# tzt101/MichiGAN

Hardware: NVIDIA H100
Metric: 512x512 images/sec (generator forward) (higher is better)
Workload: dtype fp16/bf16 tensor-core operands (bf16 hi+lo split where needed), fp32 accumulate and storage

## Files before the change

michigan_b200/csrc/mg_aux.cu:

```cuda
#include <cuda_runtime.h>
#include <cstdint>
#include <cmath>
#include <cstdlib>
#include <cuda_fp16.h>
#include <cuda_bf16.h>
#include "mg_internal.h"

namespace mg {

__device__ __forceinline__ float rtf32(float x) {
    uint32_t r;
    asm("cvt.rna.tf32.f32 %0, %1;\n" : "=r"(r) : "f"(x));
    return __uint_as_float(r);
}
__device__ __forceinline__ float act_fn(float v, int act) {
    if (act == MG_ACT_RELU) return fmaxf(v, 0.f);
    if (act == MG_ACT_LRELU) return v > 0.f ? v : 0.2f * v;
    if (act == MG_ACT_TANH) return tanhf(v);
    return v;
}
__device__ __forceinline__ void split16(float v, int fmt, uint16_t& hi, uint16_t& lo) {
    if (fmt == 1) {
        const __half h = __float2half_rn(fminf(fmaxf(v, -65504.f), 65504.f));
        hi = __half_as_ushort(h);
        lo = __half_as_ushort(__float2half_rn(v - __half2float(h)));
    } else {
        const __nv_bfloat16 h = __float2bfloat16_rn(v);
        hi = __bfloat16_as_ushort(h);
        lo = __bfloat16_as_ushort(__float2bfloat16_rn(v - __bfloat162float(h)));
    }
}
static inline int cdiv(long long a, long long b) { return (int)((a + b - 1) / b); }

__global__ void pack_weight_kernel(const float* __restrict__ w, float* __restrict__ out, int O, int I, int KH, int KW,
                                   const float* __restrict__ inv_sigma, int round_) {
    const long long total = (long long)O * KH * KW * I;
    const float s = inv_sigma ? *inv_sigma : 1.f;
    for (long long idx = blockIdx.x * (long long)blockDim.x + threadIdx.x; idx < total;
         idx += (long long)gridDim.x * blockDim.x) {
        const int i = idx % I;
        long long t = idx / I;
        const int kw = t % KW; t /= KW;
        const int kh = t % KH;
        const int o = t / KH;
        float v = w[(((long long)o * I + i) * KH + kh) * KW + kw] * s;
        out[idx] = round_ ? rtf32(v) : v;
    }
}

__global__ void pack_weight_gb_kernel(const float* __restrict__ wg, const float* __restrict__ wb,
                                      float* __restrict__ out, int C, int I, int KH, int KW, int BN) {
    const long long total = 2LL * C * KH * KW * I;
    const int half = BN / 2;
    for (long long idx = blockIdx.x * (long long)blockDim.x + threadIdx.x; idx < total;
         idx += (long long)gridDim.x * blockDim.x) {
        const int i = idx % I;
        long long t = idx / I;
        const int kw = t % KW; t /= KW;
        const int kh = t % KH;
        const int R = t / KH;
        const int tile = R / BN, rr = R % BN;
        const float* src = rr < half ? wg : wb;
        const int c = tile * half + (rr < half ? rr : rr - half);
        out[idx] = rtf32(src[(((long long)c * I + i) * KH + kh) * KW + kw]);
    }
}

__global__ void pack_weight16_kernel(const float* __restrict__ w, uint16_t* __restrict__ out, int O, int I, int KH, int KW,
                                     const float* __restrict__ inv_sigma, int fmt, int split) {
    const long long total = (long long)O * KH * KW * I;
    const float s = inv_sigma ? *inv_sigma : 1.f;
    const int parts = split ? 2 : 1;
    for (long long idx = blockIdx.x * (long long)blockDim.x + threadIdx.x; idx < total;
         idx += (long long)gridDim.x * blockDim.x) {
        const int i = idx % I;
        long long t = idx / I;
        const int kw = t % KW; t /= KW;
        const int kh = t % KH;
        const int o = t / KH;
        const float v = w[(((long long)o * I + i) * KH + kh) * KW + kw] * s;
        uint16_t hi, lo;
        split16(v, fmt, hi, lo);
        const size_t base = ((size_t)o * KH * KW + (size_t)(kh * KW + kw)) * parts * I;
        out[base + i] = hi;
        if (split) out[base + I + i] = lo;
    }
}
__global__ void pack_weight_gb16_kernel(const float* __restrict__ wg, const float* __restrict__ wb, uint16_t* __restrict__ out,
                                        int C, int I, int KH, int KW, int BN, int fmt, int split) {
// ... 109 lines not shown
                            }
                        }
#pragma unroll
                        for (int p_ = 0; p_ < 8; ++p_) {
                            const float* ip = row + (size_t)(((g * 8 + p_) * s + kw)) * CINP;
                            float iv[CINP];
                            const float4 t0 = *reinterpret_cast<const float4*>(ip);
                            iv[0] = t0.x; iv[1] = t0.y; iv[2] = t0.z; iv[3] = t0.w;
                            if constexpr (CINP == 8) {
                                const float4 t1 = *reinterpret_cast<const float4*>(ip + 4);
                                iv[4] = t1.x; iv[5] = t1.y; iv[6] = t1.z; iv[7] = t1.w;
                            }
#pragma unroll
                            for (int ci = 0; ci < CINP; ++ci)
#pragma unroll
                                for (int c = 0; c < CPL; ++c) acc[p_][c] = fmaf(iv[ci], wv[ci][c], acc[p_][c]);
                        }
                    }
                }
            }
            if (lane_active && oh < a.OH) {
                float bv[CPL];
#pragma unroll
                for (int c = 0; c < CPL; ++c) bv[c] = a.bias ? __ldg(a.bias + c_base + c) : 0.f;
#pragma unroll
                for (int p_ = 0; p_ < 8; ++p_) {
                    const int ow = ow0 + g * 8 + p_;
                    if (ow >= a.OW) continue;
                    const size_t pix = ((size_t)n * a.OH + oh) * a.OW + ow;
                    const float ps = a.pscale ? __ldg(a.pscale + pix) : 1.f;
                    const float pm = a.pmul ? __ldg(a.pmul + pix) : 1.f;
                    float y[CPL];
#pragma unroll
                    for (int c = 0; c < CPL; ++c) {
                        float v = act_fn(acc[p_][c] * ps + bv[c], a.act) * pm;
                        y[c] = a.round_out ? rtf32(v) : v;
                    }
                    if (a.out) {
                        float* op = a.out + pix * Cout + c_base;
                        if constexpr (CPL == 4) *reinterpret_cast<float4*>(op) = make_float4(y[0], y[1], y[2], y[3]);
                        else *reinterpret_cast<float2*>(op) = make_float2(y[0], y[1]);
                    }
                    if (a.out_hi) {
                        uint16_t hi[CPL], lo[CPL];
#pragma unroll
                        for (int c = 0; c < CPL; ++c) split16(y[c], a.out16_fmt, hi[c], lo[c]);
                        uint16_t* oh = reinterpret_cast<uint16_t*>(a.out_hi) + pix * Cout + c_base;
                        uint16_t* ol = a.out_lo ? reinterpret_cast<uint16_t*>(a.out_lo) + pix * Cout + c_base : nullptr;
                        if constexpr (CPL == 4) {
                            *reinterpret_cast<uint2*>(oh) = make_uint2(hi[0] | ((uint32_t)hi[1] << 16), hi[2] | ((uint32_t)hi[3] << 16));
                            if (ol) *reinterpret_cast<uint2*>(ol) = make_uint2(lo[0] | ((uint32_t)lo[1] << 16), lo[2] | ((uint32_t)lo[3] << 16));
                        } else {
                            *reinterpret_cast<uint32_t*>(oh) = hi[0] | ((uint32_t)hi[1] << 16);
                            if (ol) *reinterpret_cast<uint32_t*>(ol) = lo[0] | ((uint32_t)lo[1] << 16);
                        }
                    }
                }
            }
        }
    }
}


template <int CINP, int CPT>
__global__ void __launch_bounds__(256, 1)
thin_gemm_kernel(const mg_thin_args a, int tiles_w, int tiles_h, int num_tiles) {
    extern __shared__ __align__(16) float sm[];
    const int KH = a.KH, KW = a.KW, s = a.stride;
    constexpr int Cout = 16 * CPT;
    const int PH = 7 * s + KH, PW = 15 * s + KW;
    float* w_s = sm;
    float* in_s = sm + KH * KW * CINP * Cout;
    const int nw = KH * KW * CINP * Cout;
    for (int i = threadIdx.x * 4; i < nw; i += blockDim.x * 4)
        *reinterpret_cast<float4*>(w_s + i) = __ldg(reinterpret_cast<const float4*>(a.w + i));
    const int tx = threadIdx.x & 15, ty = threadIdx.x >> 4;
    const int prow = ty >> 1, pcol0 = (ty & 1) * 8;
    const int c_base = tx * CPT;
    const int R = a.seg_resize > 0 ? a.seg_resize : 1;
    const int IH = a.H, IW = a.W;
    float bv[CPT];
#pragma unroll
    for (int c = 0; c < CPT; ++c) bv[c] = a.bias ? __ldg(a.bias + c_base + c) : 0.f;

    for (int tile = blockIdx.x; tile < num_tiles; tile += gridDim.x) {
        const int tw = tile % tiles_w;
        const int th = (tile / tiles_w) % tiles_h;
        const int n = tile / (tiles_w * tiles_h);
        const int oh0 = th * 8, ow0 = tw * 16;
        const int ih0 = oh0 * s - a.pad, iw0 = ow0 * s - a.pad;
        __syncthreads();
        for (int i = threadIdx.x; i < PH * PW; i += blockDim.x) {
            const int py = i / PW, px = i - py * PW;
            int ih = ih0 + py, iw = iw0 + px;
            if (a.pad_mode == 1) {
                if (ih < 0) ih = -ih;
                if (ih >= IH) ih = 2 * IH - 2 - ih;
                if (iw < 0) iw = -iw;
                if (iw >= IW) iw = 2 * IW - 2 - iw;
            }
            const bool ok = ih >= 0 && ih < IH && iw >= 0 && iw < IW;
            float4 v0 = make_float4(0.f, 0.f, 0.f, 0.f), v1 = v0;
            if (ok) {
                const float* src = a.in + (((size_t)n * IH * R + (size_t)ih * R) * ((size_t)IW * R) + (size_t)iw * R) * CINP;
                v0 = __ldg(reinterpret_cast<const float4*>(src));
                if (CINP == 8) v1 = __ldg(reinterpret_cast<const float4*>(src + 4));
            }
            *reinterpret_cast<float4*>(in_s + (size_t)i * CINP) = v0;
            if (CINP == 8) *reinterpret_cast<float4*>(in_s + (size_t)i * CINP + 4) = v1;
        }
        __syncthreads();

        float acc[8][CPT];
#pragma unroll
        for (int p_ = 0; p_ < 8; ++p_)
#pragma unroll
            for (int c = 0; c < CPT; ++c) acc[p_][c] = 0.f;
        for (int kh = 0; kh < KH; ++kh) {
            const float* row = in_s + (size_t)((prow * s + kh) * PW) * CINP;
            for (int kw = 0; kw < KW; ++kw) {
                const float* wt = w_s + (size_t)((kh * KW + kw) * CINP) * Cout + c_base;
#pragma unroll
                for (int c4 = 0; c4 < CINP; c4 += 4) {
                    float wv[4][CPT];
#pragma unroll
                    for (int ci = 0; ci < 4; ++ci)
#pragma unroll
                        for (int c = 0; c < CPT; c += 4) {
                            const float4 t = *reinterpret_cast<const float4*>(wt + (size_t)(c4 + ci) * Cout + c);
                            wv[ci][c] = t.x; wv[ci][c + 1] = t.y; wv[ci][c + 2] = t.z; wv[ci][c + 3] = t.w;
                        }
#pragma unroll
                    for (int p_ = 0; p_ < 8; ++p_) {
                        const float4 iv = *reinterpret_cast<const float4*>(row + (size_t)((pcol0 + p_) * s + kw) * CINP + c4);
#pragma unroll
                        for (int c = 0; c < CPT; ++c) {
                            acc[p_][c] = fmaf(iv.x, wv[0][c], acc[p_][c]);
                            acc[p_][c] = fmaf(iv.y, wv[1][c], acc[p_][c]);
                            acc[p_][c] = fmaf(iv.z, wv[2][c], acc[p_][c]);
                            acc[p_][c] = fmaf(iv.w, wv[3][c], acc[p_][c]);
                        }
                    }
                }
            }
        }
        const int oh = oh0 + prow;
        if (oh < a.OH) {
#pragma unroll
            for (int p_ = 0; p_ < 8; ++p_) {
                const int ow = ow0 + pcol0 + p_;
                if (ow >= a.OW) continue;
                const size_t pix = ((size_t)n * a.OH + oh) * a.OW + ow;
                const float ps = a.pscale ? __ldg(a.pscale + pix) : 1.f;
                const float pm = a.pmul ? __ldg(a.pmul + pix) : 1.f;
                float y[CPT];
#pragma unroll
                for (int c = 0; c < CPT; ++c) {
                    const float v = act_fn(acc[p_][c] * ps + bv[c], a.act) * pm;
                    y[c] = a.round_out ? rtf32(v) : v;
                }
                if (a.out) {
                    float* op = a.out + pix * Cout + c_base;
#pragma unroll
                    for (int c = 0; c < CPT; c += 4) *reinterpret_cast<float4*>(op + c) = make_float4(y[c], y[c + 1], y[c + 2], y[c + 3]);
                }
                if (a.out_hi) {
                    uint16_t hi[CPT], lo[CPT];
#pragma unroll
                    for (int c = 0; c < CPT; ++c) split16(y[c], a.out16_fmt, hi[c], lo[c]);
                    uint16_t* ohp = reinterpret_cast<uint16_t*>(a.out_hi) + pix * Cout + c_base;
                    uint16_t* olp = a.out_lo ? reinterpret_cast<uint16_t*>(a.out_lo) + pix * Cout + c_base : nullptr;
#pragma unroll
                    for (int c = 0; c < CPT; c += 4) {
                        *reinterpret_cast<uint2*>(ohp + c) = make_uint2(hi[c] | ((uint32_t)hi[c + 1] << 16), hi[c + 2] | ((uint32_t)hi[c + 3] << 16));
                        if (olp) *reinterpret_cast<uint2*>(olp + c) = make_uint2(lo[c] | ((uint32_t)lo[c + 1] << 16), lo[c + 2] | ((uint32_t)lo[c + 3] << 16));
                    }
                }
            }
        }
    }
}

__global__ void __launch_bounds__(256)
conv_img_kernel(const float* __restrict__ x, const float* __restrict__ w, const float* __restrict__ bias,
                float* __restrict__ out, int N, int H, int W, int Cin, int Cout, int act_in, int act_out) {
    extern __shared__ __align__(16) float sm[];
    const int PW = 34, PH = 10, NP = PW * PH;
    const int C4 = Cin / 4;
    float* in_s = sm;
    float* w_s = sm + (size_t)C4 * NP * 4;
    for (int i = threadIdx.x; i < 9 * Cin * 4; i += blockDim.x) {
        const int co = i & 3;
        const int ci = (i >> 2) % Cin;
        const int tap = (i >> 2) / Cin;
        w_s[i] = co < Cout ? w[((size_t)co * Cin + ci) * 9 + tap] : 0.f;
    }
    const int tiles_w = (W + 31) / 32, tiles_h = (H + 7) / 8;
    const int tile = blockIdx.x;
    const int tw = tile % tiles_w, th = (tile / tiles_w) % tiles_h, n = tile / (tiles_w * tiles_h);
    const int h0 = th * 8 - 1, w0 = tw * 32 - 1;
    for (int i0 = threadIdx.x; i0 < NP * C4; i0 += 4 * blockDim.x) {
        float4 v[4];
#pragma unroll
        for (int u = 0; u < 4; ++u) {
            const int i = i0 + u * blockDim.x;
            const int c4 = i % C4, pp = i / C4;
            const int py = pp / PW, px = pp - py * PW;
            const int ih = h0 + py, iw = w0 + px;
            v[u] = make_float4(0.f, 0.f, 0.f, 0.f);
            if (i < NP * C4 && ih >= 0 && ih < H && iw >= 0 && iw < W)
                v[u] = __ldg(reinterpret_cast<const float4*>(x + (((size_t)n * H + ih) * W + iw) * Cin) + c4);
        }
#pragma unroll
        for (int u = 0; u < 4; ++u) {
            const int i = i0 + u * blockDim.x;
            if (i >= NP * C4) break;
            const int c4 = i % C4, pp = i / C4;
            const float4 r = make_float4(act_fn(v[u].x, act_in), act_fn(v[u].y, act_in), act_fn(v[u].z, act_in), act_fn(v[u].w, act_in));
            *reinterpret_cast<float4*>(in_s + ((size_t)c4 * NP + pp) * 4) = r;
        }
    }
    __syncthreads();
    const int ly = threadIdx.x >> 5, lx = threadIdx.x & 31;
    float a0 = 0.f, a1 = 0.f, a2 = 0.f;
    for (int kh = 0; kh < 3; ++kh)
        for (int kw = 0; kw < 3; ++kw) {
            const int pp = (ly + kh) * PW + lx + kw;
            const float* wt = w_s + (size_t)((kh * 3 + kw) * Cin) * 4;
// ... 863 lines not shown
```

michigan_b200/csrc/mg_wgrad.cu:

```cuda
#include <cuda.h>
#include <cuda_runtime.h>
#include <cstdio>
#include <cstring>
#include <cstdlib>
#include "mg_ptx.cuh"
#include "mg_internal.h"

namespace mg {

constexpr int kWgThreads = 288;
constexpr int kWgStagesMax = 6;
constexpr int kWgMaxCols = 256;

struct WgradParams {
    int N, OH, OW, Cout, Cin, KH, KW, stride, pad;
    int TW, TH, TN, tiles_w, tiles_h, tiles_n, pix_tiles;
    int BN, m_tiles, n_tiles, splits, stages;
    int pix_tile, box_bytes;
    int f16;
    int kelem, mboxes, kmma;
    float* dw;
    double* dw64;
};

__device__ __forceinline__ uint32_t sw128(uint32_t k, uint32_t b) {
    const uint32_t o = k * 128 + b;
    return o ^ ((k & 7) << 4);
}

__device__ __forceinline__ void mma_tf32_16x8x8(float (&c)[4], const uint32_t (&a)[4], uint32_t b0, uint32_t b1) {
    asm volatile("mma.sync.aligned.m16n8k8.row.col.f32.tf32.tf32.f32 {%0, %1, %2, %3}, {%4, %5, %6, %7}, {%8, %9}, {%0, %1, %2, %3};\n"
                 : "+f"(c[0]), "+f"(c[1]), "+f"(c[2]), "+f"(c[3])
                 : "r"(a[0]), "r"(a[1]), "r"(a[2]), "r"(a[3]), "r"(b0), "r"(b1));
}
__device__ __forceinline__ void mma_bf16_16x8x16(float (&c)[4], const uint32_t (&a)[4], uint32_t b0, uint32_t b1) {
    asm volatile("mma.sync.aligned.m16n8k16.row.col.f32.bf16.bf16.f32 {%0, %1, %2, %3}, {%4, %5, %6, %7}, {%8, %9}, {%0, %1, %2, %3};\n"
                 : "+f"(c[0]), "+f"(c[1]), "+f"(c[2]), "+f"(c[3])
                 : "r"(a[0]), "r"(a[1]), "r"(a[2]), "r"(a[3]), "r"(b0), "r"(b1));
}

template <int KWT, int BNT>
__global__ void __launch_bounds__(kWgThreads, 1)
wgrad_tf32_kernel(const __grid_constant__ CUtensorMap tmDY, const __grid_constant__ CUtensorMap tmX, const WgradParams p) {
    extern __shared__ __align__(1024) uint8_t smem_raw[];
    uint8_t* smem = reinterpret_cast<uint8_t*>((reinterpret_cast<uintptr_t>(smem_raw) + 1023) & ~uintptr_t(1023));
    const int kBoxBytes = p.box_bytes;
    const int a_bytes = p.mboxes * kBoxBytes;
    const int b1_bytes = (p.BN / p.kelem) * kBoxBytes;
    const int stage_bytes = a_bytes + p.KW * b1_bytes;
    uint64_t* bars = reinterpret_cast<uint64_t*>(smem + (size_t)p.stages * stage_bytes);
    uint64_t* full_bar = bars;
    uint64_t* empty_bar = bars + kWgStagesMax;

    const int warp = threadIdx.x >> 5, lane = threadIdx.x & 31;
    const int n_units = p.KH * p.m_tiles * p.n_tiles;
    int u = blockIdx.x % n_units;
    const int split = blockIdx.x / n_units;
    const int nt = u % p.n_tiles; u /= p.n_tiles;
    const int mt = u % p.m_tiles;
    const int kh = u / p.m_tiles;
    const int t_begin = (int)((long long)p.pix_tiles * split / p.splits);
    const int t_end = (int)((long long)p.pix_tiles * (split + 1) / p.splits);

    if (warp == 8 && lane == 0) {
        tma_prefetch_desc(&tmDY);
        tma_prefetch_desc(&tmX);
        for (int s = 0; s < p.stages; ++s) { mbar_init(&full_bar[s], 1); mbar_init(&empty_bar[s], 8); }
        fence_barrier_init();
    }
    __syncthreads();

    if (warp == 8) {
        int st = 0; uint32_t ph = 0;
        const int nb_x = p.BN / p.kelem;
        const uint32_t tx = (uint32_t)stage_bytes;
        const int n_boxes = p.mboxes + p.KW * nb_x;
        for (int t = t_begin; t < t_end; ++t) {
            const int tw = t % p.tiles_w;
            const int th = (t / p.tiles_w) % p.tiles_h;
            const int tn = t / (p.tiles_w * p.tiles_h);
            const int ow0 = tw * p.TW, oh0 = th * p.TH, n0 = tn * p.TN;
            if (lane == 0) {
                mbar_wait_report(&empty_bar[st], ph ^ 1);
                mbar_arrive_expect_tx(&full_bar[st], tx);
            }
            __syncwarp();
            uint8_t* sa = smem + (size_t)st * stage_bytes;
            for (int b = lane; b < n_boxes; b += 32) {
                if (b < p.mboxes) {
                    tma_load_4d(sa + b * kBoxBytes, &tmDY, &full_bar[st], mt * 128 + b * p.kelem, ow0, oh0, n0);
                } else {
                    const int kw = (b - p.mboxes) / nb_x, j = (b - p.mboxes) - kw * nb_x;
                    tma_load_4d(sa + a_bytes + kw * b1_bytes + j * kBoxBytes, &tmX, &full_bar[st], nt * p.BN + j * p.kelem,
                                ow0 * p.stride - p.pad + kw, oh0 * p.stride - p.pad + kh, n0);
                }
            }
            __syncwarp();
            if (++st == p.stages) { st = 0; ph ^= 1; }
        }
    } else if constexpr (KWT > 0) {
        const int wg = warp >> 2;
        float acc[KWT][BNT / 2];
#pragma unroll
        for (int kw = 0; kw < KWT; ++kw)
#pragma unroll
            for (int i = 0; i < BNT / 2; ++i) acc[kw][i] = 0.f;
        int st = 0; uint32_t ph = 0;
        for (int t = t_begin; t < t_end; ++t) {
            mbar_wait(&full_bar[st], ph);
            const uint32_t sa = smem_u32(smem + (size_t)st * stage_bytes);
            const uint32_t a_base = sa + (uint32_t)(wg * kBoxBytes), b_base = sa + (uint32_t)a_bytes;
            wgmma_fence();
#pragma unroll 1
            for (int kk = 0; kk < p.pix_tile; kk += 16) {
                const uint64_t da = wg_desc_mn_sw128(a_base + (uint32_t)(kk * 128), (uint32_t)kBoxBytes);
#pragma unroll
                for (int kw = 0; kw < KWT; ++kw) {
                    const uint64_t db = wg_desc_mn_sw128(b_base + (uint32_t)(kw * b1_bytes + kk * 128), (uint32_t)kBoxBytes);
                    if constexpr (BNT == 128) wgmma_bf16_tt_n128(acc[kw], da, db, 1u);
                    else wgmma_bf16_tt_n64(acc[kw], da, db, 1u);
                }
            }
            wgmma_commit();
            wgmma_wait_all();
            __syncwarp();
            if (lane == 0) mbar_arrive(&empty_bar[st]);
            if (++st == p.stages) { st = 0; ph ^= 1; }
        }
        if (t_end > t_begin) {
            const int r0 = mt * 128 + wg * 64 + (warp & 3) * 16 + (lane >> 2), c0 = (lane & 3) * 2;
#pragma unroll
            for (int h = 0; h < 2; ++h) {
                const int co = r0 + 8 * h;
                if (co >= p.Cout) continue;
#pragma unroll
                for (int kw = 0; kw < KWT; ++kw)
#pragma unroll
                    for (int j = 0; j < BNT / 8; ++j) {
                        const size_t off = (size_t)co * (p.KH * KWT * p.Cin) + (size_t)(kh * KWT + kw) * p.Cin + nt * BNT + j * 8 + c0;
                        const float v0 = acc[kw][4 * j + 2 * h], v1 = acc[kw][4 * j + 2 * h + 1];
                        if (p.splits > 1) {
                            atomicAdd(p.dw64 + off, (double)v0);
                            atomicAdd(p.dw64 + off + 1, (double)v1);
                        } else {
                            *reinterpret_cast<float2*>(p.dw + off) = make_float2(v0, v1);
                        }
                    }
            }
        }
    } else {
        const int g = lane >> 2, t4 = lane & 3;
        const int m0 = warp * 16;
        const int ncols = p.KW * p.BN, n8 = ncols >> 3;
        const int esz = p.f16 ? 2 : 4;
        uint32_t a_off[2];
#pragma unroll
        for (int h = 0; h < 2; ++h) {
            const int m = m0 + g + 8 * h;
            a_off[h] = (uint32_t)((m / p.kelem) * kBoxBytes) | ((uint32_t)((m % p.kelem) * esz) << 20);
        }
        float acc[kWgMaxCols / 8][4];
#pragma unroll
        for (int j = 0; j < kWgMaxCols / 8; ++j) acc[j][0] = acc[j][1] = acc[j][2] = acc[j][3] = 0.f;
        int st = 0; uint32_t ph = 0;
        for (int t = t_begin; t < t_end; ++t) {
            mbar_wait(&full_bar[st], ph);
            const uint8_t* sa = smem + (size_t)st * stage_bytes;
            auto ldA = [&](int h, int k) -> const uint8_t* { return sa + (a_off[h] & 0xFFFFF) + sw128(k, a_off[h] >> 20); };
            for (int kk = 0; kk < p.pix_tile; kk += p.kmma) {
                uint32_t a[4];
                if (p.f16) {
#pragma unroll
                    for (int i = 0; i < 4; ++i) {
                        const int h = i & 1, k = kk + 2 * t4 + 8 * (i >> 1);
                        a[i] = (uint32_t)*reinterpret_cast<const uint16_t*>(ldA(h, k)) |
                               ((uint32_t)*reinterpret_cast<const uint16_t*>(ldA(h, k + 1)) << 16);
                    }
                } else {
#pragma unroll
                    for (int i = 0; i < 4; ++i) a[i] = *reinterpret_cast<const uint32_t*>(ldA(i & 1, kk + t4 + 4 * (i >> 1)));
                }
#pragma unroll
                for (int j = 0; j < kWgMaxCols / 8; ++j) {
                    if (j < n8) {
                        const int n = j * 8 + g, kw = n / p.BN, ci = n - kw * p.BN;
                        const uint8_t* bb = sa + a_bytes + kw * b1_bytes + (ci / p.kelem) * kBoxBytes;
                        const uint32_t cb = (uint32_t)((ci % p.kelem) * esz);
                        if (p.f16) {
                            const int k = kk + 2 * t4;
                            const uint32_t b0 = (uint32_t)*reinterpret_cast<const uint16_t*>(bb + sw128(k, cb)) |
                                                ((uint32_t)*reinterpret_cast<const uint16_t*>(bb + sw128(k + 1, cb)) << 16);
                            const uint32_t b1 = (uint32_t)*reinterpret_cast<const uint16_t*>(bb + sw128(k + 8, cb)) |
                                                ((uint32_t)*reinterpret_cast<const uint16_t*>(bb + sw128(k + 9, cb)) << 16);
                            mma_bf16_16x8x16(acc[j], a, b0, b1);
                        } else {
                            const uint32_t b0 = *reinterpret_cast<const uint32_t*>(bb + sw128(kk + t4, cb));
                            const uint32_t b1 = *reinterpret_cast<const uint32_t*>(bb + sw128(kk + t4 + 4, cb));
                            mma_tf32_16x8x8(acc[j], a, b0, b1);
                        }
                    }
                }
            }
            __syncwarp();
            if (lane == 0) mbar_arrive(&empty_bar[st]);
            if (++st == p.stages) { st = 0; ph ^= 1; }
        }
        if (t_end > t_begin) {
#pragma unroll
            for (int h = 0; h < 2; ++h) {
                const int co = mt * 128 + m0 + g + 8 * h;
                if (co >= p.Cout) continue;
#pragma unroll
                for (int j = 0; j < kWgMaxCols / 8; ++j) {
                    if (j < n8) {
                        const int n = j * 8 + 2 * t4, kw = n / p.BN, ci = n - kw * p.BN;
                        const size_t off = (size_t)co * (p.KH * p.KW * p.Cin) + (size_t)(kh * p.KW + kw) * p.Cin + nt * p.BN + ci;
                        if (p.splits > 1) {
                            atomicAdd(p.dw64 + off, (double)acc[j][2 * h]);
                            atomicAdd(p.dw64 + off + 1, (double)acc[j][2 * h + 1]);
                        } else {
                            *reinterpret_cast<float2*>(p.dw + off) = make_float2(acc[j][2 * h], acc[j][2 * h + 1]);
                        }
                    }
                }
            }
        }
    }
}

static int np2(int v) { int r = 1; while (r < v) r <<= 1; return r; }

}

using namespace mg;

static int wgrad_launch(const void* dy, const void* x, float* dw, int N, int H, int W, int Cin, int OH, int OW, int Cout,
                        int KH, int KW, int stride, int pad, int fmt, cudaStream_t stream) {
    if (!dy || !x || !dw) return set_error(-1, "mg_conv_wgrad: null pointer");
    if (fmt != 0 && fmt != 2) return set_error(-5, "mg_conv_wgrad: operand format must be 0 (tf32) or 2 (bf16)");
    const int kelem = fmt ? 64 : 32;
    if (Cin % kelem != 0 || Cout % kelem != 0) return set_error(-2, "mg_conv_wgrad: channels must be multiples of %d", kelem);
    WgradParams p;
    memset(&p, 0, sizeof(p));
    p.N = N; p.OH = OH; p.OW = OW; p.Cout = Cout; p.Cin = Cin; p.KH = KH; p.KW = KW; p.stride = stride; p.pad = pad;
    p.f16 = fmt; p.kelem = kelem; p.mboxes = 128 / kelem; p.kmma = fmt ? 16 : 8;
    int BN = Cin >= 128 ? 128 : Cin;
    if (Cin % BN != 0) BN = kelem;
    while (KW * BN > kWgMaxCols) BN /= 2;
    if (BN < kelem || Cin % BN != 0) return set_error(-3, "mg_conv_wgrad: KW %d x Cin %d does not fit the accumulator", KW, Cin);
    p.BN = BN;
    int pix_tile = 64;
    if ((200 * 1024) / ((p.mboxes + KW * (BN / kelem)) * 64 * 128) < 3) pix_tile = 32;
    p.pix_tile = pix_tile; p.box_bytes = pix_tile * 128;
    p.TW = np2(OW) < 8 ? np2(OW) : 8;
    int th = pix_tile / p.TW;
    p.TH = np2(OH) < th ? np2(OH) : th;
    p.TN = pix_tile / (p.TW * p.TH);
    p.tiles_w = (OW + p.TW - 1) / p.TW; p.tiles_h = (OH + p.TH - 1) / p.TH; p.tiles_n = (N + p.TN - 1) / p.TN;
    p.pix_tiles = p.tiles_w * p.tiles_h * p.tiles_n;
    p.m_tiles = (Cout + 127) / 128;
    p.n_tiles = Cin / BN;
    const int units = KH * p.m_tiles * p.n_tiles;
    int splits = (2 * num_sms()) / units;
    if (splits < 1) splits = 1;
    if (splits > p.pix_tiles) splits = p.pix_tiles;
    p.splits = splits;
    const int stage_bytes = p.mboxes * p.box_bytes + KW * (BN / kelem) * p.box_bytes;
    int stages = (200 * 1024) / stage_bytes;
    if (stages < 1) return set_error(-4, "mg_conv_wgrad: stage of %d bytes does not fit shared memory", stage_bytes);
    if (stages > kWgStagesMax) stages = kWgStagesMax;
    p.stages = stages;
    p.dw = dw;

    CUtensorMap tmDY, tmX;
    const int esz = fmt ? 2 : 4;
    const CUtensorMapDataType dt = fmt ? CU_TENSOR_MAP_DATA_TYPE_BFLOAT16 : CU_TENSOR_MAP_DATA_TYPE_FLOAT32;
    const CUtensorMapSwizzle sw = CU_TENSOR_MAP_SWIZZLE_128B;
    {
        cuuint64_t dims[4] = {(cuuint64_t)Cout, (cuuint64_t)OW, (cuuint64_t)OH, (cuuint64_t)N};
        cuuint64_t strides[3] = {(cuuint64_t)Cout * esz, (cuuint64_t)OW * Cout * esz, (cuuint64_t)OH * OW * Cout * esz};
        cuuint32_t box[4] = {(cuuint32_t)kelem, (cuuint32_t)p.TW, (cuuint32_t)p.TH, (cuuint32_t)p.TN};
        cuuint32_t es[4] = {1, 1, 1, 1};
        int rc = encode_tensor_map(&tmDY, (void*)dy, dt, 4, dims, strides, box, es, sw);
        if (rc) return rc;
    }
    {
        cuuint64_t dims[4] = {(cuuint64_t)Cin, (cuuint64_t)W, (cuuint64_t)H, (cuuint64_t)N};
        cuuint64_t strides[3] = {(cuuint64_t)Cin * esz, (cuuint64_t)W * Cin * esz, (cuuint64_t)H * W * Cin * esz};
        cuuint32_t box[4] = {(cuuint32_t)kelem, (cuuint32_t)(p.TW * stride), (cuuint32_t)(p.TH * stride), (cuuint32_t)p.TN};
        cuuint32_t es[4] = {1, (cuuint32_t)stride, (cuuint32_t)stride, 1};
        int rc = encode_tensor_map(&tmX, (void*)x, dt, 4, dims, strides, box, es, sw);
        if (rc) return rc;
    }
    void (*kern)(CUtensorMap, CUtensorMap, WgradParams) = wgrad_tf32_kernel<0, 0>;
    if (fmt == 2) {
        if (KW == 1 && BN == 64) kern = wgrad_tf32_kernel<1, 64>;
        else if (KW == 1 && BN == 128) kern = wgrad_tf32_kernel<1, 128>;
        else if (KW == 2 && BN == 64) kern = wgrad_tf32_kernel<2, 64>;
        else if (KW == 2 && BN == 128) kern = wgrad_tf32_kernel<2, 128>;
        else if (KW == 3 && BN == 64) kern = wgrad_tf32_kernel<3, 64>;
        else if (KW == 4 && BN == 64) kern = wgrad_tf32_kernel<4, 64>;
    }
    cudaError_t e = cudaFuncSetAttribute((const void*)kern, cudaFuncAttributeMaxDynamicSharedMemorySize, 227 * 1024);
    if (e != cudaSuccess) return set_error((int)e, "wgrad attr: %s", cudaGetErrorString(e));
    const size_t smem_bytes = (size_t)stages * stage_bytes + 1024 + 256;
    const size_t n_dw = (size_t)Cout * KH * KW * Cin;
    if (splits > 1) {
        const int rc = acc64_alloc(&p.dw64, n_dw, stream);
        if (rc) return rc;
    }
    kern<<<units * splits, kWgThreads, smem_bytes, stream>>>(tmDY, tmX, p);
    int rc = check_launch("mg_conv_wgrad");
    if (splits > 1) {
        if (!rc) rc = acc64_fold(p.dw64, dw, n_dw, 0, stream);
        const int rc2 = acc64_free(p.dw64, stream);
        if (!rc) rc = rc2;
    }
    return rc;
}

extern "C" int mg_conv_wgrad(const float* dy, const float* x, float* dw, int N, int H, int W, int Cin, int OH, int OW, int Cout,
                             int KH, int KW, int stride, int pad, void* stream_) {
    return wgrad_launch(dy, x, dw, N, H, W, Cin, OH, OW, Cout, KH, KW, stride, pad, 0, reinterpret_cast<cudaStream_t>(stream_));
}

extern "C" int mg_conv_wgrad16(const void* dy16, const void* x16, float* dw, int N, int H, int W, int Cin, int OH, int OW, int Cout,
                               int KH, int KW, int stride, int pad, void* stream_) {
    return wgrad_launch(dy16, x16, dw, N, H, W, Cin, OH, OW, Cout, KH, KW, stride, pad, 2, reinterpret_cast<cudaStream_t>(stream_));
}
```

Before: 201.7.

## Skip zero last input channel in thin conv and move TF32 wgrad to wgmma

The thin direct-convolution kernel now checks whether the last padded input channel's weights are all zero and, if so, runs a compile-time variant that skips those FMAs. Separately, the TF32 weight-gradient kernel replaces its mma.sync fallback with a wgmma path: TMA lands tiles in a ring, and consumer warps transpose them into double-buffered K-major stages before issuing wgmma. The wgrad change only matters for backward passes, so it probably does not affect the generator-forward metric. It adds shared-memory transposes, and it fails with an error for any KW/BN combination that has no compiled variant.

```diff
diff --git a/michigan_b200/csrc/mg_aux.cu b/michigan_b200/csrc/mg_aux.cu
--- a/michigan_b200/csrc/mg_aux.cu
+++ b/michigan_b200/csrc/mg_aux.cu
@@ -5,6 +5,7 @@
 #include <cuda_fp16.h>
 #include <cuda_bf16.h>
 #include "mg_internal.h"
+#include <type_traits>
 
 namespace mg {
 
@@ -280,6 +281,12 @@
     float bv[CPT];
 #pragma unroll
     for (int c = 0; c < CPT; ++c) bv[c] = a.bias ? __ldg(a.bias + c_base + c) : 0.f;
+    bool last_nz = false;
+    for (int i = threadIdx.x; i < KH * KW * Cout; i += blockDim.x) {
+        const int tap = i / Cout, c = i - tap * Cout;
+        last_nz |= __ldg(a.w + (size_t)(tap * CINP + CINP - 1) * Cout + c) != 0.f;
+    }
+    const bool skip_last = !__syncthreads_or(last_nz);
 
     for (int tile = blockIdx.x; tile < num_tiles; tile += gridDim.x) {
         const int tw = tile % tiles_w;
@@ -314,34 +321,39 @@
         for (int p_ = 0; p_ < 8; ++p_)
 #pragma unroll
             for (int c = 0; c < CPT; ++c) acc[p_][c] = 0.f;
-        for (int kh = 0; kh < KH; ++kh) {
-            const float* row = in_s + (size_t)((prow * s + kh) * PW) * CINP;
-            for (int kw = 0; kw < KW; ++kw) {
-                const float* wt = w_s + (size_t)((kh * KW + kw) * CINP) * Cout + c_base;
-#pragma unroll
-                for (int c4 = 0; c4 < CINP; c4 += 4) {
-                    float wv[4][CPT];
-#pragma unroll
-                    for (int ci = 0; ci < 4; ++ci)
-#pragma unroll
-                        for (int c = 0; c < CPT; c += 4) {
-                            const float4 t = *reinterpret_cast<const float4*>(wt + (size_t)(c4 + ci) * Cout + c);
-                            wv[ci][c] = t.x; wv[ci][c + 1] = t.y; wv[ci][c + 2] = t.z; wv[ci][c + 3] = t.w;
-                        }
-#pragma unroll
-                    for (int p_ = 0; p_ < 8; ++p_) {
-                        const float4 iv = *reinterpret_cast<const float4*>(row + (size_t)((pcol0 + p_) * s + kw) * CINP + c4);
-#pragma unroll
-                        for (int c = 0; c < CPT; ++c) {
-                            acc[p_][c] = fmaf(iv.x, wv[0][c], acc[p_][c]);
-                            acc[p_][c] = fmaf(iv.y, wv[1][c], acc[p_][c]);
-                            acc[p_][c] = fmaf(iv.z, wv[2][c], acc[p_][c]);
-                            acc[p_][c] = fmaf(iv.w, wv[3][c], acc[p_][c]);
+        auto mac = [&](auto nci) {
+            constexpr int NCI = decltype(nci)::value;
+            for (int kh = 0; kh < KH; ++kh) {
+                const float* row = in_s + (size_t)((prow * s + kh) * PW) * CINP;
+                for (int kw = 0; kw < KW; ++kw) {
+                    const float* wt = w_s + (size_t)((kh * KW + kw) * CINP) * Cout + c_base;
+#pragma unroll
+                    for (int c4 = 0; c4 < CINP; c4 += 4) {
+                        float wv[4][CPT];
+#pragma unroll
+                        for (int ci = 0; ci < 4; ++ci)
+#pragma unroll
+                            for (int c = 0; c < CPT; c += 4) {
+                                if (c4 + ci >= NCI) continue;
+                                const float4 t = *reinterpret_cast<const float4*>(wt + (size_t)(c4 + ci) * Cout + c);
+                                wv[ci][c] = t.x; wv[ci][c + 1] = t.y; wv[ci][c + 2] = t.z; wv[ci][c + 3] = t.w;
+                            }
+#pragma unroll
+                        for (int p_ = 0; p_ < 8; ++p_) {
+                            const float4 iv = *reinterpret_cast<const float4*>(row + (size_t)((pcol0 + p_) * s + kw) * CINP + c4);
+                            const float ivs[4] = {iv.x, iv.y, iv.z, iv.w};
+#pragma unroll
+                            for (int c = 0; c < CPT; ++c)
+#pragma unroll
+                                for (int ci = 0; ci < 4; ++ci)
+                                    if (c4 + ci < NCI) acc[p_][c] = fmaf(ivs[ci], wv[ci][c], acc[p_][c]);
                         }
                     }
                 }
             }
-        }
+        };
+        if (skip_last) mac(std::integral_constant<int, CINP - 1>{});
+        else mac(std::integral_constant<int, CINP>{});
         const int oh = oh0 + prow;
         if (oh < a.OH) {
 #pragma unroll
diff --git a/michigan_b200/csrc/mg_wgrad.cu b/michigan_b200/csrc/mg_wgrad.cu
--- a/michigan_b200/csrc/mg_wgrad.cu
+++ b/michigan_b200/csrc/mg_wgrad.cu
@@ -11,54 +11,69 @@
 constexpr int kWgThreads = 288;
 constexpr int kWgStagesMax = 6;
 constexpr int kWgMaxCols = 256;
+constexpr int kWgSmemBudget = 200 * 1024;
+constexpr int kWgTf32Box = 32 * 128;
 
 struct WgradParams {
-    int N, OH, OW, Cout, Cin, KH, KW, stride, pad;
+    int N, OH, OW, Cout, Cin, KH, stride, pad;
     int TW, TH, TN, tiles_w, tiles_h, tiles_n, pix_tiles;
-    int BN, m_tiles, n_tiles, splits, stages;
+    int m_tiles, n_tiles, splits, stages;
     int pix_tile, box_bytes;
-    int f16;
-    int kelem, mboxes, kmma;
+    int kelem, mboxes;
     float* dw;
     double* dw64;
 };
 
-__device__ __forceinline__ uint32_t sw128(uint32_t k, uint32_t b) {
-    const uint32_t o = k * 128 + b;
-    return o ^ ((k & 7) << 4);
-}
-
-__device__ __forceinline__ void mma_tf32_16x8x8(float (&c)[4], const uint32_t (&a)[4], uint32_t b0, uint32_t b1) {
-    asm volatile("mma.sync.aligned.m16n8k8.row.col.f32.tf32.tf32.f32 {%0, %1, %2, %3}, {%4, %5, %6, %7}, {%8, %9}, {%0, %1, %2, %3};\n"
-                 : "+f"(c[0]), "+f"(c[1]), "+f"(c[2]), "+f"(c[3])
-                 : "r"(a[0]), "r"(a[1]), "r"(a[2]), "r"(a[3]), "r"(b0), "r"(b1));
-}
-__device__ __forceinline__ void mma_bf16_16x8x16(float (&c)[4], const uint32_t (&a)[4], uint32_t b0, uint32_t b1) {
-    asm volatile("mma.sync.aligned.m16n8k16.row.col.f32.bf16.bf16.f32 {%0, %1, %2, %3}, {%4, %5, %6, %7}, {%8, %9}, {%0, %1, %2, %3};\n"
-                 : "+f"(c[0]), "+f"(c[1]), "+f"(c[2]), "+f"(c[3])
-                 : "r"(a[0]), "r"(a[1]), "r"(a[2]), "r"(a[3]), "r"(b0), "r"(b1));
-}
-
-template <int KWT, int BNT>
+template <int KW, int BN>
+struct WgTf32 {
+    static constexpr int boxes = 4 + KW * (BN / 32);
+    static constexpr int stage_bytes = boxes * kWgTf32Box;
+    static constexpr int kmajor = 2;
+    static constexpr int fit = kWgSmemBudget / stage_bytes - kmajor;
+    static constexpr int landing = fit < kWgStagesMax ? fit : kWgStagesMax;
+    static_assert(landing >= 2, "TF32 wgrad stage does not fit two landing + two K-major stages");
+};
+
+__device__ __forceinline__ void lds128(uint32_t (&v)[4], uint32_t addr) {
+    asm volatile("ld.shared.v4.b32 {%0, %1, %2, %3}, [%4];\n" : "=r"(v[0]), "=r"(v[1]), "=r"(v[2]), "=r"(v[3]) : "r"(addr) : "memory");
+}
+__device__ __forceinline__ void sts128(uint32_t addr, uint32_t a, uint32_t b, uint32_t c, uint32_t d) {
+    asm volatile("st.shared.v4.b32 [%0], {%1, %2, %3, %4};\n" ::"r"(addr), "r"(a), "r"(b), "r"(c), "r"(d) : "memory");
+}
+
+struct WgUnit { int nt, mt, kh, split; };
+__device__ __forceinline__ WgUnit wg_unit(const WgradParams& p) {
+    uint32_t b;
+    asm volatile("mov.u32 %0, %%ctaid.x;\n" : "=r"(b));
+    const int n_units = p.KH * p.m_tiles * p.n_tiles;
+    int u = (int)b % n_units;
+    WgUnit r;
+    r.split = (int)b / n_units;
+    r.nt = u % p.n_tiles; u /= p.n_tiles;
+    r.mt = u % p.m_tiles;
+    r.kh = u / p.m_tiles;
+    return r;
+}
+
+template <int FMT, int KWT, int BNT>
 __global__ void __launch_bounds__(kWgThreads, 1)
 wgrad_tf32_kernel(const __grid_constant__ CUtensorMap tmDY, const __grid_constant__ CUtensorMap tmX, const WgradParams p) {
+    static_assert(FMT == 0 || FMT == 2, "operand format");
+    static_assert(KWT * BNT <= kWgMaxCols, "accumulator");
     extern __shared__ __align__(1024) uint8_t smem_raw[];
     uint8_t* smem = reinterpret_cast<uint8_t*>((reinterpret_cast<uintptr_t>(smem_raw) + 1023) & ~uintptr_t(1023));
     const int kBoxBytes = p.box_bytes;
     const int a_bytes = p.mboxes * kBoxBytes;
-    const int b1_bytes = (p.BN / p.kelem) * kBoxBytes;
-    const int stage_bytes = a_bytes + p.KW * b1_bytes;
-    uint64_t* bars = reinterpret_cast<uint64_t*>(smem + (size_t)p.stages * stage_bytes);
+    const int b1_bytes = (BNT / p.kelem) * kBoxBytes;
+    const int stage_bytes = a_bytes + KWT * b1_bytes;
+    uint8_t* ring = smem + (FMT == 0 ? 2 * stage_bytes : 0);
+    uint64_t* bars = reinterpret_cast<uint64_t*>(ring + (size_t)p.stages * stage_bytes);
     uint64_t* full_bar = bars;
     uint64_t* empty_bar = bars + kWgStagesMax;
 
     const int warp = threadIdx.x >> 5, lane = threadIdx.x & 31;
-    const int n_units = p.KH * p.m_tiles * p.n_tiles;
-    int u = blockIdx.x % n_units;
-    const int split = blockIdx.x / n_units;
-    const int nt = u % p.n_tiles; u /= p.n_tiles;
-    const int mt = u % p.m_tiles;
-    const int kh = u / p.m_tiles;
+    const WgUnit un = wg_unit(p);
+    const int split = un.split, nt = un.nt, mt = un.mt, kh = un.kh;
     const int t_begin = (int)((long long)p.pix_tiles * split / p.splits);
     const int t_end = (int)((long long)p.pix_tiles * (split + 1) / p.splits);
 
@@ -72,9 +87,9 @@
 
     if (warp == 8) {
         int st = 0; uint32_t ph = 0;
-        const int nb_x = p.BN / p.kelem;
+        const int nb_x = BNT / p.kelem;
         const uint32_t tx = (uint32_t)stage_bytes;
-        const int n_boxes = p.mboxes + p.KW * nb_x;
+        const int n_boxes = p.mboxes + KWT * nb_x;
         for (int t = t_begin; t < t_end; ++t) {
             const int tw = t % p.tiles_w;
             const int th = (t / p.tiles_w) % p.tiles_h;
@@ -85,20 +100,20 @@
                 mbar_arrive_expect_tx(&full_bar[st], tx);
             }
             __syncwarp();
-            uint8_t* sa = smem + (size_t)st * stage_bytes;
+            uint8_t* sa = ring + (size_t)st * stage_bytes;
             for (int b = lane; b < n_boxes; b += 32) {
                 if (b < p.mboxes) {
                     tma_load_4d(sa + b * kBoxBytes, &tmDY, &full_bar[st], mt * 128 + b * p.kelem, ow0, oh0, n0);
                 } else {
                     const int kw = (b - p.mboxes) / nb_x, j = (b - p.mboxes) - kw * nb_x;
-                    tma_load_4d(sa + a_bytes + kw * b1_bytes + j * kBoxBytes, &tmX, &full_bar[st], nt * p.BN + j * p.kelem,
+                    tma_load_4d(sa + a_bytes + kw * b1_bytes + j * kBoxBytes, &tmX, &full_bar[st], nt * BNT + j * p.kelem,
                                 ow0 * p.stride - p.pad + kw, oh0 * p.stride - p.pad + kh, n0);
                 }
             }
             __syncwarp();
             if (++st == p.stages) { st = 0; ph ^= 1; }
         }
-    } else if constexpr (KWT > 0) {
+    } else {
         const int wg = warp >> 2;
         float acc[KWT][BNT / 2];
 #pragma unroll
@@ -106,28 +121,82 @@
 #pragma unroll
             for (int i = 0; i < BNT / 2; ++i) acc[kw][i] = 0.f;
         int st = 0; uint32_t ph = 0;
-        for (int t = t_begin; t < t_end; ++t) {
-            mbar_wait(&full_bar[st], ph);
-            const uint32_t sa = smem_u32(smem + (size_t)st * stage_bytes);
-            const uint32_t a_base = sa + (uint32_t)(wg * kBoxBytes), b_base = sa + (uint32_t)a_bytes;
-            wgmma_fence();
+        if constexpr (FMT == 2) {
+            for (int t = t_begin; t < t_end; ++t) {
+                mbar_wait(&full_bar[st], ph);
+                const uint32_t sa = smem_u32(ring + (size_t)st * stage_bytes);
+                const uint32_t a_base = sa + (uint32_t)(wg * kBoxBytes), b_base = sa + (uint32_t)a_bytes;
+                wgmma_fence();
 #pragma unroll 1
-            for (int kk = 0; kk < p.pix_tile; kk += 16) {
-                const uint64_t da = wg_desc_mn_sw128(a_base + (uint32_t)(kk * 128), (uint32_t)kBoxBytes);
-#pragma unroll
-                for (int kw = 0; kw < KWT; ++kw) {
-                    const uint64_t db = wg_desc_mn_sw128(b_base + (uint32_t)(kw * b1_bytes + kk * 128), (uint32_t)kBoxBytes);
-                    if constexpr (BNT == 128) wgmma_bf16_tt_n128(acc[kw], da, db, 1u);
-                    else wgmma_bf16_tt_n64(acc[kw], da, db, 1u);
+                for (int kk = 0; kk < p.pix_tile; kk += 16) {
+                    const uint64_t da = wg_desc_mn_sw128(a_base + (uint32_t)(kk * 128), (uint32_t)kBoxBytes);
+#pragma unroll
+                    for (int kw = 0; kw < KWT; ++kw) {
+                        const uint64_t db = wg_desc_mn_sw128(b_base + (uint32_t)(kw * b1_bytes + kk * 128), (uint32_t)kBoxBytes);
+                        if constexpr (BNT == 128) wgmma_bf16_tt_n128(acc[kw], da, db, 1u);
+                        else wgmma_bf16_tt_n64(acc[kw], da, db, 1u);
+                    }
                 }
-            }
-            wgmma_commit();
-            wgmma_wait_all();
-            __syncwarp();
-            if (lane == 0) mbar_arrive(&empty_bar[st]);
-            if (++st == p.stages) { st = 0; ph ^= 1; }
+                wgmma_commit();
+                wgmma_wait_all();
+                __syncwarp();
+                if (lane == 0) mbar_arrive(&empty_bar[st]);
+                if (++st == p.stages) { st = 0; ph ^= 1; }
+            }
+        } else {
+            using G = WgTf32<KWT, BNT>;
+            constexpr int kBlocks = G::boxes * 64;
+            const int kq = threadIdx.x & 7, cq = kq ^ ((threadIdx.x >> 3) & 7);
+            const uint32_t box0 = (threadIdx.x >> 6) * kWgTf32Box;
+            const uint32_t ld0 = box0 + kq * 512 + ((cq ^ (4 * (kq & 1))) << 4);
+            const uint32_t st0 = box0 + cq * 512 + ((kq ^ (4 * (cq & 1))) << 4);
+            const uint32_t kmaj = smem_u32(smem);
+            const uint32_t land = smem_u32(ring);
+            auto transpose = [&](int ks) {
+                mbar_wait(&full_bar[st], ph);
+                const uint32_t src = land + (uint32_t)(st * G::stage_bytes) + ld0;
+                const uint32_t dst = kmaj + (uint32_t)(ks * G::stage_bytes) + st0;
+#pragma unroll 1
+                for (int it = 0; it < (kBlocks + 255) / 256; ++it) {
+                    if (kBlocks % 256 == 0 || (int)threadIdx.x + 256 * it < kBlocks) {
+                        const uint32_t o = (uint32_t)(it * 4 * kWgTf32Box);
+                        uint32_t v[4][4];
+#pragma unroll
+                        for (int i = 0; i < 4; ++i) lds128(v[i], ((src + o) + 128 * i) ^ (16 * i));
+#pragma unroll
+                        for (int j = 0; j < 4; ++j) sts128(((dst + o) + 128 * j) ^ (16 * j), v[0][j], v[1][j], v[2][j], v[3][j]);
+                    }
+                }
+                fence_proxy_async_smem();
+                __syncwarp();
+                if (lane == 0) mbar_arrive(&empty_bar[st]);
+                if (++st == p.stages) { st = 0; ph ^= 1; }
+            };
+            const int steps = t_end - t_begin;
+            if (steps > 0) transpose(0);
+            for (int i = 0; i < steps; ++i) {
+                const int ks = i & 1;
+                bar_sync(1, 256);
+                const uint32_t a = kmaj + (uint32_t)(ks * G::stage_bytes + wg * 64 * 128);
+                const uint32_t b = kmaj + (uint32_t)(ks * G::stage_bytes + 4 * kWgTf32Box);
+                wgmma_fence();
+#pragma unroll
+                for (int k = 0; k < 4; ++k) {
+                    const uint64_t da = wg_desc_sw128(a + (uint32_t)(32 * k), 1024);
+#pragma unroll
+                    for (int kw = 0; kw < KWT; ++kw)
+                        wgmma_step<0, BNT>(acc[kw], da, wg_desc_sw128(b + (uint32_t)(kw * BNT * 128 + 32 * k), 1024), 1u);
+                }
+                wgmma_commit();
+                if (i + 1 < steps) transpose(ks ^ 1);
+                wgmma_wait<0>();
+            }
+#pragma unroll
+            for (int kw = 0; kw < KWT; ++kw) wgmma_fence_operand(acc[kw]);
         }
         if (t_end > t_begin) {
+            const WgUnit eu = FMT == 0 ? wg_unit(p) : un;
+            const int mt = eu.mt, kh = eu.kh, nt = eu.nt;
             const int r0 = mt * 128 + wg * 64 + (warp & 3) * 16 + (lane >> 2), c0 = (lane & 3) * 2;
 #pragma unroll
             for (int h = 0; h < 2; ++h) {
@@ -148,84 +217,36 @@
                     }
             }
         }
-    } else {
-        const int g = lane >> 2, t4 = lane & 3;
-        const int m0 = warp * 16;
-        const int ncols = p.KW * p.BN, n8 = ncols >> 3;
-        const int esz = p.f16 ? 2 : 4;
-        uint32_t a_off[2];
-#pragma unroll
-        for (int h = 0; h < 2; ++h) {
-            const int m = m0 + g + 8 * h;
-            a_off[h] = (uint32_t)((m / p.kelem) * kBoxBytes) | ((uint32_t)((m % p.kelem) * esz) << 20);
-        }
-        float acc[kWgMaxCols / 8][4];
-#pragma unroll
-        for (int j = 0; j < kWgMaxCols / 8; ++j) acc[j][0] = acc[j][1] = acc[j][2] = acc[j][3] = 0.f;
-        int st = 0; uint32_t ph = 0;
-        for (int t = t_begin; t < t_end; ++t) {
-            mbar_wait(&full_bar[st], ph);
-            const uint8_t* sa = smem + (size_t)st * stage_bytes;
-            auto ldA = [&](int h, int k) -> const uint8_t* { return sa + (a_off[h] & 0xFFFFF) + sw128(k, a_off[h] >> 20); };
-            for (int kk = 0; kk < p.pix_tile; kk += p.kmma) {
-                uint32_t a[4];
-                if (p.f16) {
-#pragma unroll
-                    for (int i = 0; i < 4; ++i) {
-                        const int h = i & 1, k = kk + 2 * t4 + 8 * (i >> 1);
-                        a[i] = (uint32_t)*reinterpret_cast<const uint16_t*>(ldA(h, k)) |
-                               ((uint32_t)*reinterpret_cast<const uint16_t*>(ldA(h, k + 1)) << 16);
-                    }
-                } else {
-#pragma unroll
-                    for (int i = 0; i < 4; ++i) a[i] = *reinterpret_cast<const uint32_t*>(ldA(i & 1, kk + t4 + 4 * (i >> 1)));
-                }
-#pragma unroll
-                for (int j = 0; j < kWgMaxCols / 8; ++j) {
-                    if (j < n8) {
-                        const int n = j * 8 + g, kw = n / p.BN, ci = n - kw * p.BN;
-                        const uint8_t* bb = sa + a_bytes + kw * b1_bytes + (ci / p.kelem) * kBoxBytes;
-                        const uint32_t cb = (uint32_t)((ci % p.kelem) * esz);
-                        if (p.f16) {
-                            const int k = kk + 2 * t4;
-                            const uint32_t b0 = (uint32_t)*reinterpret_cast<const uint16_t*>(bb + sw128(k, cb)) |
-                                                ((uint32_t)*reinterpret_cast<const uint16_t*>(bb + sw128(k + 1, cb)) << 16);
-                            const uint32_t b1 = (uint32_t)*reinterpret_cast<const uint16_t*>(bb + sw128(k + 8, cb)) |
-                                                ((uint32_t)*reinterpret_cast<const uint16_t*>(bb + sw128(k + 9, cb)) << 16);
-                            mma_bf16_16x8x16(acc[j], a, b0, b1);
-                        } else {
-                            const uint32_t b0 = *reinterpret_cast<const uint32_t*>(bb + sw128(kk + t4, cb));
-                            const uint32_t b1 = *reinterpret_cast<const uint32_t*>(bb + sw128(kk + t4 + 4, cb));
-                            mma_tf32_16x8x8(acc[j], a, b0, b1);
-                        }
-                    }
-                }
-            }
-            __syncwarp();
-            if (lane == 0) mbar_arrive(&empty_bar[st]);
-            if (++st == p.stages) { st = 0; ph ^= 1; }
-        }
-        if (t_end > t_begin) {
-#pragma unroll
-            for (int h = 0; h < 2; ++h) {
-                const int co = mt * 128 + m0 + g + 8 * h;
-                if (co >= p.Cout) continue;
-#pragma unroll
-                for (int j = 0; j < kWgMaxCols / 8; ++j) {
-                    if (j < n8) {
-                        const int n = j * 8 + 2 * t4, kw = n / p.BN, ci = n - kw * p.BN;
-                        const size_t off = (size_t)co * (p.KH * p.KW * p.Cin) + (size_t)(kh * p.KW + kw) * p.Cin + nt * p.BN + ci;
-                        if (p.splits > 1) {
-                            atomicAdd(p.dw64 + off, (double)acc[j][2 * h]);
-                            atomicAdd(p.dw64 + off + 1, (double)acc[j][2 * h + 1]);
-                        } else {
-                            *reinterpret_cast<float2*>(p.dw + off) = make_float2(acc[j][2 * h], acc[j][2 * h + 1]);
-                        }
-                    }
-                }
-            }
-        }
-    }
+    }
+}
+
+typedef void (*WgradKernel)(CUtensorMap, CUtensorMap, WgradParams);
+
+template <int KW, int BN>
+static WgradKernel tf32_variant(int* landing) {
+    *landing = WgTf32<KW, BN>::landing;
+    return wgrad_tf32_kernel<0, KW, BN>;
+}
+
+static WgradKernel wgrad_variant(int fmt, int KW, int BN, int* landing) {
+    if (fmt == 0) {
+        if (KW == 1 && BN == 32) return tf32_variant<1, 32>(landing);
+        if (KW == 1 && BN == 64) return tf32_variant<1, 64>(landing);
+        if (KW == 1 && BN == 128) return tf32_variant<1, 128>(landing);
+        if (KW == 3 && BN == 32) return tf32_variant<3, 32>(landing);
+        if (KW == 3 && BN == 64) return tf32_variant<3, 64>(landing);
+        if (KW == 4 && BN == 32) return tf32_variant<4, 32>(landing);
+        if (KW == 4 && BN == 64) return tf32_variant<4, 64>(landing);
+        if (KW == 7 && BN == 32) return tf32_variant<7, 32>(landing);
+        return nullptr;
+    }
+    if (KW == 1 && BN == 64) return wgrad_tf32_kernel<2, 1, 64>;
+    if (KW == 1 && BN == 128) return wgrad_tf32_kernel<2, 1, 128>;
+    if (KW == 2 && BN == 64) return wgrad_tf32_kernel<2, 2, 64>;
+    if (KW == 2 && BN == 128) return wgrad_tf32_kernel<2, 2, 128>;
+    if (KW == 3 && BN == 64) return wgrad_tf32_kernel<2, 3, 64>;
+    if (KW == 4 && BN == 64) return wgrad_tf32_kernel<2, 4, 64>;
+    return nullptr;
 }
 
 static int np2(int v) { int r = 1; while (r < v) r <<= 1; return r; }
@@ -242,15 +263,17 @@
     if (Cin % kelem != 0 || Cout % kelem != 0) return set_error(-2, "mg_conv_wgrad: channels must be multiples of %d", kelem);
     WgradParams p;
     memset(&p, 0, sizeof(p));
-    p.N = N; p.OH = OH; p.OW = OW; p.Cout = Cout; p.Cin = Cin; p.KH = KH; p.KW = KW; p.stride = stride; p.pad = pad;
-    p.f16 = fmt; p.kelem = kelem; p.mboxes = 128 / kelem; p.kmma = fmt ? 16 : 8;
+    p.N = N; p.OH = OH; p.OW = OW; p.Cout = Cout; p.Cin = Cin; p.KH = KH; p.stride = stride; p.pad = pad;
+    p.kelem = kelem; p.mboxes = 128 / kelem;
     int BN = Cin >= 128 ? 128 : Cin;
     if (Cin % BN != 0) BN = kelem;
     while (KW * BN > kWgMaxCols) BN /= 2;
     if (BN < kelem || Cin % BN != 0) return set_error(-3, "mg_conv_wgrad: KW %d x Cin %d does not fit the accumulator", KW, Cin);
-    p.BN = BN;
+    int landing = 0;
+    const WgradKernel kern = wgrad_variant(fmt, KW, BN, &landing);
+    if (!kern) return set_error(-6, "mg_conv_wgrad: no compiled %s variant for KW %d x BN %d", fmt ? "bf16" : "tf32", KW, BN);
     int pix_tile = 64;
-    if ((200 * 1024) / ((p.mboxes + KW * (BN / kelem)) * 64 * 128) < 3) pix_tile = 32;
+    if (fmt == 0 || kWgSmemBudget / ((p.mboxes + KW * (BN / kelem)) * 64 * 128) < 3) pix_tile = 32;
     p.pix_tile = pix_tile; p.box_bytes = pix_tile * 128;
     p.TW = np2(OW) < 8 ? np2(OW) : 8;
     int th = pix_tile / p.TW;
@@ -266,7 +289,7 @@
     if (splits > p.pix_tiles) splits = p.pix_tiles;
     p.splits = splits;
     const int stage_bytes = p.mboxes * p.box_bytes + KW * (BN / kelem) * p.box_bytes;
-    int stages = (200 * 1024) / stage_bytes;
+    int stages = fmt == 0 ? landing : kWgSmemBudget / stage_bytes;
     if (stages < 1) return set_error(-4, "mg_conv_wgrad: stage of %d bytes does not fit shared memory", stage_bytes);
     if (stages > kWgStagesMax) stages = kWgStagesMax;
     p.stages = stages;
@@ -292,18 +315,9 @@
         int rc = encode_tensor_map(&tmX, (void*)x, dt, 4, dims, strides, box, es, sw);
         if (rc) return rc;
     }
-    void (*kern)(CUtensorMap, CUtensorMap, WgradParams) = wgrad_tf32_kernel<0, 0>;
-    if (fmt == 2) {
-        if (KW == 1 && BN == 64) kern = wgrad_tf32_kernel<1, 64>;
-        else if (KW == 1 && BN == 128) kern = wgrad_tf32_kernel<1, 128>;
-        else if (KW == 2 && BN == 64) kern = wgrad_tf32_kernel<2, 64>;
-        else if (KW == 2 && BN == 128) kern = wgrad_tf32_kernel<2, 128>;
-        else if (KW == 3 && BN == 64) kern = wgrad_tf32_kernel<3, 64>;
-        else if (KW == 4 && BN == 64) kern = wgrad_tf32_kernel<4, 64>;
-    }
     cudaError_t e = cudaFuncSetAttribute((const void*)kern, cudaFuncAttributeMaxDynamicSharedMemorySize, 227 * 1024);
     if (e != cudaSuccess) return set_error((int)e, "wgrad attr: %s", cudaGetErrorString(e));
-    const size_t smem_bytes = (size_t)stages * stage_bytes + 1024 + 256;
+    const size_t smem_bytes = (size_t)(stages + (fmt == 0 ? 2 : 0)) * stage_bytes + 1024 + 256;
     const size_t n_dw = (size_t)Cout * KH * KW * Cin;
     if (splits > 1) {
         const int rc = acc64_alloc(&p.dw64, n_dw, stream);
```

Result: no change. 202.9 (median of 6 runs) (+0.6%).
